# jeremy-collins/sd-video-gen

Measured on AMD Instinct MI355X. Metric: generated frames/sec at 50 DDIM denoise steps, 512x512, higher is better.
Workload: dtype fp16; 1 GPU; configs[2]: 1_16_kitti_L1_64 F=64, 64x64 latents -> 512x512 VAE passes, 50-step DDIM; --denoise --denoise_start_step 0, guidance_scale 0; SD-v1.4 UNet at 64x64 latents, VAE enc/dec at 512x512; clips_per_gpu=56, streams_per_gpu=2, pred_frames=1, global_clips=56, parallelism=clip-sharded dp1, weights=seeded random init (SD v1.4 architecture, 1_16_kitti_L1_64)

## Files before the change

sd-video-gen_amd/csrc/attn.hip:

```cpp
#include "kernels.h"
#include "igemm_epi.h"
#include <cstdlib>

namespace SDNS {

typedef float f32x16 __attribute__((ext_vector_type(16)));

namespace {

constexpr int KVT = 64;
constexpr int VROW = 136;

__device__ __forceinline__ float max3(float a, float b, float c) {
  float r;
  asm("v_max3_f32 %0, %1, %2, %3" : "=v"(r) : "v"(a), "v"(b), "v"(c));
  return r;
}
__device__ __forceinline__ float max_xor32(float v) {
  const auto r = __builtin_amdgcn_permlane32_swap(__float_as_uint(v), __float_as_uint(v), false, false);
  return fmaxf(__uint_as_float(r[0]), __uint_as_float(r[1]));
}

template <int D, int QB, int NSTW, bool BC, bool HV = false>
__global__ void __launch_bounds__(256) attn_kernel(const AttnArgs a) {
// ... 389 lines not shown
      *(uint4*)(sK + tid * KROW + 80) = make_uint4(H16_ONE2, H16_ONE1, 0, 0);
      *(uint4*)(sK + tid * KROW + 96) = make_uint4(0, 0, 0, 0);
    }
    for (int i = tid; i < 24 * 8; i += 256) {
      const int row = 40 + i / 8, pos = i & 7;
      *(uint4*)(sV + row * 128 + pos * 16) = row == 40 ? make_uint4(H16_ONE2, H16_ONE2, H16_ONE2, H16_ONE2) : make_uint4(0, 0, 0, 0);
    }
  }
  __syncthreads();

  f32x16 O[QB][DVT];
  float m_run[QB];
  constexpr float TAU = 6.f;
#pragma unroll
  for (int qb = 0; qb < QB; ++qb) {
#pragma unroll
    for (int i = 0; i < DVT; ++i)
#pragma unroll
      for (int j = 0; j < 16; ++j) O[qb][i][j] = 0.f;
    m_run[qb] = 0.f;
  }

  issue(0);
  if (ntiles > 1) issue(1);
  for (int t = 0; t < ntiles; ++t) {
    if (t + 1 < ntiles) asm volatile("s_waitcnt vmcnt(3)" ::: "memory");
    else asm volatile("s_waitcnt vmcnt(0)" ::: "memory");
    __syncthreads();
    if (t + 2 < ntiles) issue(t + 2);
    const char* const sK = smem + (t % DM_NST) * STAGE;
    const char* const sV = sK + K_BYTES;

    f32x16 S0[QB], S1[QB];
#pragma unroll
    for (int qb = 0; qb < QB; ++qb)
#pragma unroll
      for (int j = 0; j < 16; ++j) { S0[qb][j] = 0.f; S1[qb][j] = 0.f; }
#ifndef ATTN_PRIO
#define ATTN_PRIO 0
#endif
    if (ATTN_PRIO & 1) __builtin_amdgcn_s_setprio(1);
#pragma unroll
    for (int ks = 0; ks < KS; ++ks) {
      const h16x8 a0 = *(const h16x8*)(sK + r * KROW + (ks * 2 + h) * 16);
      const h16x8 a1 = *(const h16x8*)(sK + (32 + r) * KROW + (ks * 2 + h) * 16);
#pragma unroll
      for (int qb = 0; qb < QB; ++qb) {
        S0[qb] = MFMA_32x32x16(a0, qf[qb][ks], S0[qb]);
        S1[qb] = MFMA_32x32x16(a1, qf[qb][ks], S1[qb]);
      }
    }
    if (ATTN_PRIO & 1) __builtin_amdgcn_s_setprio(0);
    uint4 vfr[4 * DVT];
#pragma unroll
    for (int i = 0; i < 4; ++i)
#pragma unroll
      for (int dt = 0; dt < DVT; ++dt) {
        const int row = 32 * dt + r;
        vfr[i * DVT + dt] = *(const uint4*)(sV + row * 128 + (((2 * i + h) ^ ((row >> 1) & 7)) << 4));
      }
    __builtin_amdgcn_sched_barrier(0);
    if (t * KVT + KVT > a.Skv) {
      const int base = t * KVT + 8 * h;
#pragma unroll
      for (int qb = 0; qb < QB; ++qb)
#pragma unroll
        for (int j = 0; j < 16; ++j) {
          const int kv = 16 * (j >> 3) + 4 * ((j >> 2) & 1) + (j & 3);
          if (base + kv >= a.Skv) S0[qb][j] = -INFINITY;
          if (base + 32 + kv >= a.Skv) S1[qb][j] = -INFINITY;
        }
    }
    if (ATTN_PRIO & 4) __builtin_amdgcn_s_setprio(1);
    float mx[QB];
#pragma unroll
    for (int qb = 0; qb < QB; ++qb) {
      float v = fmaxf(S0[qb][0], S1[qb][0]);
#pragma unroll
      for (int j = 1; j < 16; ++j) v = max3(v, S0[qb][j], S1[qb][j]);
      mx[qb] = max_xor32(v);
    }
#pragma unroll
    for (int qb = 0; qb < QB; ++qb) {
      if (t == 0 || __any(mx[qb] > TAU)) {
        const float delta = (t == 0 || mx[qb] > 0.f) ? mx[qb] : 0.f;
        const float alpha = __builtin_amdgcn_exp2f(-delta);
        m_run[qb] += delta;
#pragma unroll
        for (int i = 0; i < DVT; ++i)
#pragma unroll
          for (int j = 0; j < 16; ++j) O[qb][i][j] *= alpha;
#pragma unroll
        for (int j = 0; j < 16; ++j) { S0[qb][j] -= delta; S1[qb][j] -= delta; }
        const float v0 = -m_run[qb];
        const h16 p1 = (h16)v0;
        const float r1 = v0 - (float)p1;
        const h16 p2 = (h16)r1;
        const h16 p3 = (h16)(r1 - (float)p2);
        if (h == 1) { qf[qb][KS - 1][0] = p1; qf[qb][KS - 1][1] = p2; qf[qb][KS - 1][2] = p3; }
      }
#pragma unroll
      for (int j = 0; j < 16; ++j) {
        S0[qb][j] = __builtin_amdgcn_exp2f(S0[qb][j]);
        S1[qb][j] = __builtin_amdgcn_exp2f(S1[qb][j]);
      }
    }
    if (ATTN_PRIO & 4) __builtin_amdgcn_s_setprio(0);
#pragma unroll
    for (int st = 0; st < 2; ++st)
#pragma unroll
      for (int s2 = 0; s2 < 2; ++s2) {
        h16x8 pf[QB];
#pragma unroll
        for (int qb = 0; qb < QB; ++qb)
#pragma unroll
          for (int j = 0; j < 8; ++j) pf[qb][j] = (h16)(st == 0 ? S0[qb][8 * s2 + j] : S1[qb][8 * s2 + j]);
        if (ATTN_PRIO & 2) __builtin_amdgcn_s_setprio(1);
#pragma unroll
        for (int dt = 0; dt < DVT; ++dt) {
          const uint4 v = vfr[(2 * st + s2) * DVT + dt];
#pragma unroll
          for (int qb = 0; qb < QB; ++qb)
            O[qb][dt] = MFMA_32x32x16(*(const h16x8*)&v, pf[qb], O[qb][dt]);
        }
        if (ATTN_PRIO & 2) __builtin_amdgcn_s_setprio(0);
      }
  }

#pragma unroll
  for (int qb = 0; qb < QB; ++qb) {
    const float l_tot = __shfl(O[qb][LT][LR], r + 32 * LH);
    const float inv = 1.f / l_tot;
    const int q = q0 + 32 * qb + r;
    if (q < a.Sq) {
      h16* orow = a.out + (int64_t)b * a.ob + (int64_t)q * a.ldo + head * D;
#pragma unroll
      for (int dt = 0; dt < DVT; ++dt)
#pragma unroll
        for (int g = 0; g < 4; ++g) {
          const int dd = 32 * dt + 8 * g + 4 * h;
          if (dd < D) {
            h16x4 w;
            w[0] = (h16)(O[qb][dt][4 * g + 0] * inv);
            w[1] = (h16)(O[qb][dt][4 * g + 1] * inv);
            w[2] = (h16)(O[qb][dt][4 * g + 2] * inv);
            w[3] = (h16)(O[qb][dt][4 * g + 3] * inv);
            *(h16x4*)(orow + dd) = w;
          }
        }
    }
  }
}

template <int D>
void launch(const AttnPath& p, const AttnArgs& a, hipStream_t s) {
  constexpr bool CAN_BC = (D % 16) == 8;
  if constexpr (D == 40) {
    if (p.kernel == ATTN_DMA40) {
      hipLaunchKernelGGL(attn_dma40_kernel, dim3(cdiv(a.Sq, 256) * a.heads * a.B), dim3(256), 0, s, a);
      return;
    }
  }
  if constexpr (D <= 64) {
    if (p.qb == 2) {
      const dim3 grid(cdiv(a.Sq, 256) * a.heads * a.B);
      if constexpr (CAN_BC) {
        if (p.bc && p.hv) { hipLaunchKernelGGL((attn_kernel<D, 2, 1, true, true>), grid, dim3(256), 0, s, a); return; }
        if (p.bc) { hipLaunchKernelGGL((attn_kernel<D, 2, 1, true>), grid, dim3(256), 0, s, a); return; }
      }
      if (p.nst == 2) hipLaunchKernelGGL((attn_kernel<D, 2, 2, false>), grid, dim3(256), 0, s, a);
      else hipLaunchKernelGGL((attn_kernel<D, 2, 1, false>), grid, dim3(256), 0, s, a);
      return;
    }
  }
  const dim3 grid(cdiv(a.Sq, 128) * a.heads * a.B);
  if constexpr (CAN_BC) {
    if (p.bc) { hipLaunchKernelGGL((attn_kernel<D, 1, 1, true>), grid, dim3(256), 0, s, a); return; }
  }
  if constexpr (D != 160) {
    if (p.nst == 2) { hipLaunchKernelGGL((attn_kernel<D, 1, 2, false>), grid, dim3(256), 0, s, a); return; }
  }
  hipLaunchKernelGGL((attn_kernel<D, 1, 1, false>), grid, dim3(256), 0, s, a);
}

int attn_stages(int d) {
  const int dk = (d + 15) / 16 * 16, dvt = (d + 31) / 32;
  const int stage = KVT * (dk * 2 + 16) + dvt * 32 * VROW;
  return 2 * stage <= 65536 ? 2 : 1;
}

bool attn_d_supported(int d) {
  switch (d) { case 8: case 16: case 32: case 40: case 64: case 80: case 160: return true; default: return false; }
}

bool attn_path_exists(const AttnPath& p) {
  const int d = p.d;
  if (!attn_d_supported(d)) return false;
  if (p.kernel == ATTN_DMA40) return d == 40 && p.qb == 2 && p.nst == 3 && p.bc == 1 && p.hv == 1;
  if (p.kernel != ATTN_REG) return false;
  if (p.qb != 1 && !(p.qb == 2 && d <= 64)) return false;
  if (p.bc) return (d % 16) == 8 && p.bc == 1 && p.nst == 1 && (p.hv == 0 || (p.hv == 1 && p.qb == 2));
  return p.hv == 0 && (p.nst == 1 || (p.nst == 2 && attn_stages(d) == 2));
}

}

AttnPath attention_describe(const AttnArgs& a, const AttnPath* force) {
  SVG_CHECK(attn_d_supported(a.d), "attention: head dim %d unsupported (instantiated: 8, 16, 32, 40, 64, 80, 160)", a.d);
  if (force) {
    SVG_CHECK(force->d == a.d && attn_path_exists(*force), "attention: no instantiation {kernel %d, d %d, QB %d, NST %d, BC %d, HV %d} for d = %d",
              force->kernel, force->d, force->qb, force->nst, force->bc, force->hv, a.d);
    return *force;
  }
  const int nst_env = (int)svg_env_i64("SVG_ATTN_NST", 1);
  const int qb_env = (int)svg_env_i64("SVG_ATTN_QB", 2);
  const int bc_env = (int)svg_env_i64("SVG_ATTN_BC", 1);
  const int hv_env = (int)svg_env_i64("SVG_ATTN_HV", 1);
  const int dma_env = (int)svg_env_i64("SVG_ATTN_DMA", 1);
  const int d = a.d;
  const bool can_bc = (d % 16) == 8;
  AttnPath p;
  p.d = d;
  if (d == 40 && dma_env && qb_env == 2 && bc_env && a.Sq >= 512) {
    p.kernel = ATTN_DMA40; p.qb = 2; p.nst = 3; p.bc = 1; p.hv = 1;
    return p;
  }
  p.qb = (d <= 64 && qb_env == 2 && a.Sq >= 512) ? 2 : 1;
  if (can_bc && bc_env) { p.bc = 1; p.hv = (p.qb == 2 && hv_env) ? 1 : 0; }
  else if (nst_env == 2) p.nst = attn_stages(d);
  return p;
}

void attention(svg_ctx* ctx, const AttnArgs& a, hipStream_t s, const AttnPath* force, AttnPath* ran) {
  SVG_CHECK(a.ldq % 8 == 0 && a.ldk % 8 == 0 && a.ldvt % 8 == 0 && a.ldo % 4 == 0, "attention: strides must be 16-byte aligned");
  SVG_CHECK(a.ldvt >= (a.Skv + 7) / 8 * 8, "attention: V^T rows must be padded to a multiple of 8 keys");
  SVG_CHECK(a.Skv > 0 && a.Sq > 0, "attention: empty");
  const AttnPath p = attention_describe(a, force);
  if (ran) *ran = p;
  if (!SVG_LAUNCHING(ctx)) return;
  char tag[128];
  if (p.kernel == ATTN_DMA40) snprintf(tag, sizeof(tag), "B%d_h%d_Sq%d_Skv%d_d%d_dma40", a.B, a.heads, a.Sq, a.Skv, a.d);
  else snprintf(tag, sizeof(tag), "B%d_h%d_Sq%d_Skv%d_d%d_qb%d_nst%d_bc%d_hv%d", a.B, a.heads, a.Sq, a.Skv, a.d, p.qb, p.nst, p.bc, p.hv);
  ProfScope ps(ctx, PK_ATTN, s, 4.0 * a.B * a.heads * (double)a.Sq * a.Skv * a.d,
               2.0 * a.B * a.heads * ((double)a.Sq * a.d * 2 + (double)a.Skv * a.d * 2), tag);
  switch (a.d) {
    case 8: launch<8>(p, a, s); break;
    case 16: launch<16>(p, a, s); break;
    case 32: launch<32>(p, a, s); break;
    case 40: launch<40>(p, a, s); break;
    case 64: launch<64>(p, a, s); break;
    case 80: launch<80>(p, a, s); break;
    case 160: launch<160>(p, a, s); break;
    default: SVG_CHECK(false, "attention: head dim %d unsupported (instantiated: 8, 16, 32, 40, 64, 80, 160)", a.d);
  }
  check_launch("attention");
}

}
```

sd-video-gen_amd/csrc/kernels.h:

```cpp
#pragma once
#include "common.h"
#include "gemm_tiles.h"

namespace SDNS {

enum AMode { A_DENSE = 0, A_CONV_S1 = 1, A_CONV_S2P1 = 2, A_CONV_S2ASYM = 3, A_CONV_UP2 = 4, A_CONV_SMALLC = 5 };
enum Act { ACT_NONE = 0, ACT_SILU = 1, ACT_GELU = 2, ACT_GEGLU = 3 };

struct GemmArgs {
  const h16* A = nullptr;
  int amode = A_DENSE;
  int lda = 0;
  const h16* A2 = nullptr;
  int lda2 = 0, k_split = 0;
  int H = 0, W = 0, Cin = 0;
  int Ho = 0, Wo = 0;
  const h16* Wt = nullptr;
  int ldb = 0;
  int n_valid = 0;
  void* C = nullptr;
  int ldc = 0;
  int M = 0, N = 0, K = 0;
  int batch = 1;
  int64_t sA = 0, sB = 0, sC = 0;
  float alpha = 1.f;
  const float* bias = nullptr;
  int bias_row = 0;
  const float* bias_bn = nullptr;
  int rows_per_batch = 1;
  int bias_bn_ld = 0;
  const h16* residual = nullptr;
  int ldr = 0;
  int act = ACT_NONE;
  int out_f32 = 0;
  const float* ln_rs = nullptr;
  const float* ln_rm = nullptr;
  const float* ln_s = nullptr;
  int ln_swapped = 0;
  int64_t ln_zstride = 0;
  int splitk = 1;
  float* slabs = nullptr;
  float* gn_part = nullptr;
  float* ln_part = nullptr;
  int ln_tiles = 0;
  int64_t bias_zs = 0;
  h16* vt_out = nullptr;
  int vt_n0 = 0, vt_rows = 0, vt_ld = 0;
  int64_t vt_bs = 0;
  int tn_major = 0;
  int group_m = 0;
  int pp_merge = 0;
  int pp_dma_m = 0;
  int dbg = 0;
  const float* residual_f32 = nullptr;
};

enum GemmFamily { GF_IGEMM = 0, GF_HALO = 1, GF_PP = 2, GF_WS = 3 };
struct GemmPlan {
  int family = GF_IGEMM, bn = 0, splitk = 1;
  int gn_rows = 0;
  int ln_tiles = 0;
  bool operator==(const GemmPlan& o) const { return family == o.family && bn == o.bn && splitk == o.splitk && gn_rows == o.gn_rows && ln_tiles == o.ln_tiles; }
};
GemmPlan gemm_plan(const GemmArgs& g);
void gemm_auto(svg_ctx* ctx, GemmArgs g, const GemmPlan& plan, hipStream_t s, int prof_kind);
void gemm_auto(svg_ctx* ctx, GemmArgs g, hipStream_t s, int prof_kind);
void launch_conv_halo(const GemmArgs& g, int bn, dim3 grid, hipStream_t s);
void launch_gemm_ws(svg_ctx* ctx, const GemmArgs& g, int group_cols, hipStream_t s);
void launch_gemm_pp(const GemmArgs& g, int bn, hipStream_t s);
void gemm_init_device();
void gemm_pp_init_device();
void gemm_ws_init_device();
void conv_halo_init_device();
void ff_fused_init_device();
void xattn_fused_init_device();
void gemm_fp8_init_device();

void quant_mx_h16(svg_ctx* ctx, const h16* x, int ldx, uint8_t* q, uint8_t* sc, int64_t rows, int K, hipStream_t s);
void quant_mx_f32(const float* x, int ldx, uint8_t* q, uint8_t* sc, int64_t rows, int K, hipStream_t s);
bool gemm_fp8_supported(int M, int N, int K);
void gemm_fp8(svg_ctx* ctx, const uint8_t* A, const uint8_t* As, const uint8_t* W, const uint8_t* Ws, const GemmArgs& g, hipStream_t s,
              int* bn_used = nullptr);

bool conv_halo_fp8_supported(int B, int H, int W, int Cin, int N);
void conv_halo_fp8_init_device();
void quant_act_mx(svg_ctx* ctx, const h16* x, int C, uint8_t* q, uint8_t* sc, int64_t P, hipStream_t s);
void pack_conv3x3_mx(const float* w_oihw, uint8_t* q, uint8_t* sc, int O, int I, int Npad, int Cp, hipStream_t s);
struct Fp8ConvPath { int bn = 0, tn_major = 0, workgroups = 0; };
void conv_halo_fp8(svg_ctx* ctx, const uint8_t* A8, const uint8_t* As, const uint8_t* W8, const uint8_t* Ws, int Npad, const GemmArgs& g, hipStream_t s,
                   Fp8ConvPath* path = nullptr);

bool ff_fused_supported(int C, int M);
bool xattn_fused_supported(int C, int heads, int M, int rows_per_sample, int L);
int64_t xattn_kv_pack_elems(int N);
void xattn_pack_q(const float* w, const float* gamma, const float* beta, h16* Wq, float* sq, float* bq, int perm, hipStream_t s);
bool xattn_chain_enabled();
void xattn_pack_o(const float* w, h16* Wo, hipStream_t s);
void xattn_pack_kv(const h16* K, int ldk, int64_t k_bs, const h16* Vt, int ldv, int64_t v_bs, h16* Kp, h16* Vp, int N, int L, hipStream_t s);
void xattn_fused(svg_ctx* ctx, const h16* X, int ldx, const h16* R, int ldr, const h16* Wp, const float* bp, const float* rs, const float* rm,
                 const h16* Wq, const float* sq, const float* bq, const h16* Kp, const h16* Vp, const h16* Wo, const float* bo, h16* out, int ldo,
                 int M, int rows_per_sample, int L, hipStream_t s);
void pack_ff2_perm(const float* w, h16* out, int N, int K, hipStream_t s);
void ff_fused(svg_ctx* ctx, const h16* X, int ldx, const h16* W1, const float* b1, const float* s1,
              const h16* W2p, const float* b2, const h16* residual, int ldr, h16* out, int ldo, int M, hipStream_t s);
void pack_conv3x3(const float* w_oihw, h16* out, int O, int I, int Opad, int Ipad, hipStream_t s);
void pack_linear(const float* w, h16* out, int N, int K, int Npad, hipStream_t s);
void fold_ln_weights(float* w, const float* bias_in, const float* gamma, const float* beta, float* bias_out, int N, int K, hipStream_t s);
void rowsum_h16(const h16* w, float* out, int N, int K, hipStream_t s);
void ln_stats(svg_ctx* ctx, const h16* x, float* rs, float* rm, int M, int C, float eps, hipStream_t s);
void pack_geglu(const float* w, const float* b, h16* wout, float* bout, int F, int K, hipStream_t s);

void ln_finish(svg_ctx* ctx, const float* part, int tiles, float* rs, float* rm, int M, int C, float eps, hipStream_t s);
struct GnStats {
  const float* part = nullptr;
  int tiles_per_sample = 0;
  bool valid() const { return part != nullptr && tiles_per_sample > 0; }
};
void groupnorm(svg_ctx* ctx, const h16* x, int C1, const h16* x2, int C2, const float* gamma,
               const float* beta, h16* out, int B, int HW, int groups, float eps, int silu,
               hipStream_t s, const GnStats* st1 = nullptr, const GnStats* st2 = nullptr);
void groupnorm_f32(svg_ctx* ctx, const float* x, int C, const float* gamma, const float* beta, h16* out, int B, int HW, int groups, float eps,
                   int silu, hipStream_t s, const GnStats* st = nullptr);
enum GnKind { GN_NONE = -1, GN_SMALL = 0, GN_STATS_APPLY = 1, GN_FINISH_APPLY = 2, GN_FINISH_APPLY_MX = 3 };
struct GnPath {
  int kind = GN_NONE, maxch = 0, vw = 0;
  int CV = 0, PL = 0, nchunk = 0, nblk = 0, threads = 0;
};
struct GnShape {
  int C1 = 0, C2 = 0, B = 0, HW = 0, groups = 0;
  bool f32_in = false;
  bool have_stats = false;
  bool mx_out = false;
};
bool groupnorm_mx(svg_ctx* ctx, const h16* x, int C1, const h16* x2, int C2, const float* gamma, const float* beta, uint8_t* q, uint8_t* sc,
                  int B, int HW, int groups, float eps, int silu, hipStream_t s, const GnStats* st1, const GnStats* st2,
                  float* stats_out = nullptr, GnPath* ran = nullptr);
GnPath groupnorm_describe(const GnShape& a, const GnPath* force = nullptr);
void groupnorm_ex(svg_ctx* ctx, const void* x, int C1, const void* x2, int C2, bool f32_in, const float* gamma, const float* beta, h16* out,
                  int B, int HW, int groups, float eps, int silu, hipStream_t s, const GnStats* st1, const GnStats* st2, const GnPath* force,
                  GnPath* ran);
void gn_finish(svg_ctx* ctx, const GnStats& st1, int C1, const GnStats* st2, int C2, float* stats, int B, int HW, int groups, float eps,
               hipStream_t s);
void gn_fold_weights(const float* W, const float* bias, const float* gamma, const float* beta, const float* stats, h16* Wb,
                     float* bb, int B, int N, int C, int groups, hipStream_t s);
void layernorm(svg_ctx* ctx, const h16* x, const float* gamma, const float* beta, h16* out, int M,
               int C, float eps, hipStream_t s);
void softmax_rows(svg_ctx* ctx, const float* s_in, h16* p_out, int64_t rows, int cols, int ld_in,
                  int ld_out, float scale, hipStream_t s);

struct AttnArgs {
  const h16 *q, *k, *vt;
  h16* out;
  int B, heads, Sq, Skv, d;
  int ldq, ldk, ldvt, ldo;
  int64_t qb, kb, vtb, ob;
  float scale;
};
enum AttnKernel { ATTN_REG = 0, ATTN_DMA40 = 1 };
struct AttnPath {
  int kernel = ATTN_REG, d = 0, qb = 1, nst = 1, bc = 0, hv = 0;
};
AttnPath attention_describe(const AttnArgs& a, const AttnPath* force = nullptr);
void attention(svg_ctx* ctx, const AttnArgs& a, hipStream_t s, const AttnPath* force = nullptr, AttnPath* ran = nullptr);
bool vae_attention_supported(int S, int C, int ldqk, int ldvt, int ldo);
bool vae_attention_shape_ok(int S, int C, int ldqk, int ldvt, int ldo);
void vae_attention(svg_ctx* ctx, const h16* q, const h16* k, int ldqk, int64_t qkb, const h16* vt, int ldvt, int64_t vtb, h16* out, int ldo,
                   int64_t ob, int B, int S, int C, hipStream_t s);
void vae_attn_init_device();

void img_to_act(const uint8_t* img, h16* out, int N, int sh, int sw, int H, int W, hipStream_t s);
void act_to_img(const float* x, int ldc, uint8_t* img, float* fout, int N, int h, int w, int oh, int ow,
                hipStream_t s);
void nchw_to_act(const float* x, h16* out, int N, int C, int h, int w, int Cpad, float scale, hipStream_t s);
void nchw_to_actf32(const float* x, float* out, int N, int C, int h, int w, float scale, hipStream_t s);
void actf32_pad_h16(const float* x, int C, h16* out, int Cpad, int64_t P, hipStream_t s);
void actf32_to_nchw(const float* x, int ld, float* out, int N, int C, int h, int w, hipStream_t s);
void pixel_linear_f32(const float* x, int ldx, const float* w, const float* b, float* y, int ldy,
                      int64_t P, int Cin, int Cout, hipStream_t s);
void vae_sample(const float* mom, int ldm, const float* eps_nchw, float* z_nchw, float* mom_nchw, int N,
                int h, int w, hipStream_t s);
void concat_channels(const h16* a, int Ca, const h16* b, int Cb, h16* out, int64_t P, hipStream_t s);
void resize_bilinear_f32(const float* src, float* dst, int P, int h, int w, int oh, int ow, hipStream_t s);
void resize_nearest_u8(const uint8_t* src, uint8_t* dst, int N, int sh, int sw, int C, int dh, int dw,
                       hipStream_t s);
void f32_to_h16(const float* x, h16* y, int64_t n, hipStream_t s);
void h16_to_f32(const h16* x, float* y, int64_t n, hipStream_t s);
void f32_to_h16_x8(const float* x, h16* y, int64_t n, hipStream_t s);
void timestep_embed(const float* t, h16* out, int N, int dim, hipStream_t s);
void fill_f32(float* p, int64_t n, float v, hipStream_t s);

}

void xf_train_init_device();
void xformer_init_device();

struct XfGemmPath { int form, mt, ksplit; };
XfGemmPath xf_gemm_describe(int M, int N, int K);
void xf_gemm(svg_ctx* ctx, const float* X, const float* W, const float* bias, float* Y, int M, int N,
             int K, int act_in, hipStream_t s, const float* residual = nullptr, XfGemmPath* ran = nullptr);
void xf_embed_tokens(const int32_t* ids, const float* tok, const float* pos, float* y, int rows, int T, int d, int vocab, hipStream_t s);
void xf_attention_causal(const float* qkv, float* o, int B, int T, int heads, int hd, hipStream_t s);
void xf_attention_padded(const float* qkv, const int32_t* lens, float* o, int B, int T, int heads, int hd, hipStream_t s);
void xf_embed_bert(const int32_t* ids, const float* word, const float* pos, const float* type0, float* y, int rows, int T, int d, int vocab,
                   hipStream_t s);
void xf_mean_pool_norm(const float* x, const int32_t* lens, float* out, int B, int T, int d, hipStream_t s);
void xf_add_ln(const float* x, const float* r, const float* g, const float* b, float* y, int M, int d,
               float eps, hipStream_t s);
void xf_embed_post(const float* emb, const float* pe, const int32_t* pe_row, const float* text, int d_txt, float* y, int B, int T,
                   int d, float scale, hipStream_t s);
struct XfDrop { const uint64_t* seed; uint32_t site; float p; };
struct XfAdamTensor { float* p; const float* g; float* m; float* v; };
struct XfAdamChunk { int32_t ten; int32_t n; int64_t off; };
void xf_drop_mask(const XfDrop d, float* out, int64_t n, hipStream_t s);
void xf_gemm_tn(const float* dY, int ldy, const float* X, int ldx, float* dW, float* db, int M, int N, int K, int accumulate, hipStream_t s);
int64_t xf_gemm_nn_slab_floats(int M, int N, int K);
int xf_gemm_nn_splits(int N, int K);
void xf_gemm_nn(const float* dY, int ldy, const float* W, float* slabs, float* out, int M, int N, int K, const float* gate, float gate_scale,
                const float* add, hipStream_t s);
void xf_relu_drop(const float* h, float* r, int64_t n, const XfDrop d, hipStream_t s);
void xf_add_ln_train(const float* x, const float* r, const XfDrop dr, const float* g, const float* b, float* y, float* xhat, float* rstd, int M,
                     int d, float eps, hipStream_t s);
void xf_ln_bwd(const float* dy, const float* xhat, const float* rstd, const float* g, float* dz, float* dz_drop, const XfDrop dr, float* dgamma,
               float* dbeta, int M, int d, int accumulate, hipStream_t s);
void xf_embed_post_train(const float* emb, const float* pe, const int32_t* pe_row, const float* text, int d_txt, float* y, int B, int T, int d,
                         float scale, const XfDrop dr, hipStream_t s);
void xf_embed_post_bwd(const float* dy, float* de, int B, int T, int d, int d_img, float scale, const XfDrop dr, hipStream_t s);
void xf_attention_train(const float* q, int ldq, const float* k, const float* v, int ldk, const float* mask, float* o, float* P, int Tq, int Tk,
                        int B, int heads, int hd, const XfDrop dr, hipStream_t s);
void xf_attention_bwd(const float* dout, const float* q, int ldq, const float* k, const float* v, int ldk, const float* P, float* dq, int lddq,
                      float* dk, float* dv, int lddk, int Tq, int Tk, int B, int heads, int hd, const XfDrop dr, hipStream_t s);
void xf_criterion(const float* pred, const float* expected, float* dpred, float* part, float* part2, float* losses, int Tt, int B, int D, int t0,
                  int fh, int fw, float w_mse, float w_l1, float w_gdl, float alpha, float w_nce, float temperature, hipStream_t s);
void xf_adam(const XfAdamTensor* tens, const XfAdamChunk* chunks, int n_chunks, float lr, float beta1, float beta2, float eps, int step,
             float* const* ema, float ema_decay, hipStream_t s);
void xf_grad_norm(const XfAdamTensor* tens, const XfAdamChunk* chunks, int n_chunks, double* part, double* norm, hipStream_t s);
void xf_adamw(const XfAdamTensor* tens, const XfAdamChunk* chunks, int n_chunks, float lr, float beta1, float beta2, float eps, int step,
              float weight_decay, int decoupled, float grad_scale, float max_norm, const double* norm, float* const* ema, float ema_decay,
              hipStream_t s);
void xf_attention(const float* q, int ldq, const float* k, const float* v, int ldk, const float* mask,
                  float* o, int Tq, int Tk, int B, int heads, int hd, hipStream_t s, const float* kpad = nullptr);

int64_t frame_metrics_tiles(int H, int W);
void frame_metrics(const uint8_t* a, const uint8_t* b, int N, int H, int W, double* part_ssim, uint32_t* part_sse, int64_t* sse, double* ssim,
                   float* ssim_map, hipStream_t s);

struct Conv3dArgs {
  const float* x; int B, T, H, W, Cin;
  const float* w;
  const float* bias;
  float* y; int To, Ho, Wo, Cout, ldc, coff;
  int kt, kh, kw, st, sh, sw, pt, ph, pw;
  int relu;
};
void conv3d_launch(const Conv3dArgs& a, hipStream_t s);
void pack_conv3d(const float* w, const float* gamma, const float* beta, const float* mean, const float* var, const float* cbias, float* wout,
                 float* bout, int Cout, int Cin, int Cin_pad, int taps, float eps, hipStream_t s);
void maxpool3d_same(const float* x, float* y, int B, int T, int H, int W, int C, int To, int Ho, int Wo, const int k[3], const int st[3],
                    const int pf[3], hipStream_t s);
void avgpool_thw(const float* x, float* y, int B, int T, int HW, int C, int kt, hipStream_t s);
void time_mean(const float* x, float* y, int B, int To, int C, hipStream_t s);
void ncthw_to_nthwc(const float* x, float* y, int B, int C, int T, int H, int W, int Cp, hipStream_t s);
void fvd_preprocess(const uint8_t* v, float* out, int B, int T, int H, int W, int res, hipStream_t s);
void fd_moments(const float* x, int n, int d, double* mean, double* cov, hipStream_t s);
void sym_eig(double* A, double* V, int d, double* cs, hipStream_t s);
void frechet_distance(const float* x1, int n1, const float* x2, int n2, int d, double* ws, double* out, hipStream_t s);
```

sd-video-gen_amd/csrc/sdnet.cpp:

```cpp
#include "models.h"
#include <algorithm>
#include <cstdlib>

namespace SDNS {

static int64_t chunk_limit() {
  const int64_t full = (1LL << 31) - 1;
  const int64_t v = svg_env_i64("SVG_CHUNK_LIMIT", full);
  return v > 0 && v < full ? v : full;
}

float* keep_f32(svg_ctx* ctx, WeightStore& ws, const std::string& name, int64_t numel) {
  const Weight& w = ws.get(name);
  SVG_CHECK(w.numel == numel, "weight %s has %lld elements, expected %lld", name.c_str(), (long long)w.numel, (long long)numel);
  return w.f32;
}

ConvW load_conv3x3(svg_ctx* ctx, WeightStore& ws, const std::string& prefix, int Cin, int Cout, hipStream_t s, bool fp8) {
  const Weight& w = ws.get(prefix + ".weight", {Cout, Cin, 3, 3});
  ConvW cw;
  cw.Cout = Cout;
  cw.Opad = (int)align_up(Cout, 4);
  cw.Cin = (Cin < 64) ? 8 : Cin;
  SVG_CHECK(Cin <= 8 || Cin % 64 == 0, "conv %s: Cin=%d must be <= 8 or a multiple of 64", prefix.c_str(), Cin);
// ... 78 lines not shown

ConvDims conv_out_dims(int amode, int H, int W) {
  switch (amode) {
    case A_CONV_S1: return {H, W};
    case A_CONV_S2P1: case A_CONV_S2ASYM: return {H / 2, W / 2};
    case A_CONV_UP2: return {2 * H, 2 * W};
    default: throw SvgError("conv3x3: bad mode");
  }
}

bool conv3x3_fp8_ok(const ConvW& cw, int B, int H, int W, bool up2) {
  return cw.w8 != nullptr && conv_halo_fp8_supported(B, up2 ? 2 * H : H, up2 ? 2 * W : W, cw.Cin, cw.Opad);
}

GemmArgs conv3x3_fp8_args(const ConvW& cw, h16* out, int B, int H, int W, int amode, const ConvOpts& o) {
  SVG_CHECK((amode == A_CONV_S1 || amode == A_CONV_UP2) && !o.out_f32 && !o.residual_f32, "conv3x3_fp8: stride 1 (mode %d), 16-bit output and residual only", amode);
  SVG_CHECK(conv3x3_fp8_ok(cw, B, H, W, amode == A_CONV_UP2), "conv3x3_fp8: %d x %dx%d x %d -> %d does not qualify", B, H, W, cw.Cin, cw.Opad);
  const ConvDims d = conv_out_dims(amode, H, W);
  GemmArgs g;
  g.H = H; g.W = W; g.Cin = cw.Cin; g.amode = amode; g.Ho = d.Ho; g.Wo = d.Wo;
  g.K = 9 * cw.Cin; g.M = B * d.Ho * d.Wo; g.N = cw.Opad; g.n_valid = cw.Opad;
  g.bias = cw.b;
  g.bias_bn = o.bias_bn; g.bias_bn_ld = o.bias_bn_ld; g.rows_per_batch = d.Ho * d.Wo;
  g.residual = o.residual; g.ldr = cw.Opad;
  g.C = out; g.ldc = cw.Opad;
  return g;
}

void conv3x3_fp8(svg_ctx* ctx, const uint8_t* x8, const uint8_t* xs, const ConvW& cw, h16* out, int B, int H, int W, int amode, hipStream_t s,
                 const ConvOpts& o) {
  GemmArgs g = conv3x3_fp8_args(cw, out, B, H, W, amode, o);
  attach_gn_emit(g, o.emit, g.Ho * g.Wo, 256);
  conv_halo_fp8(ctx, x8, xs, cw.w8, cw.w8s, cw.Opad, g, s);
}

GemmArgs conv3x3_args(const h16* x, const ConvW& cw, int B, int H, int W, int amode, int out_f32) {
  GemmArgs g;
  g.A = x; g.H = H; g.W = W; g.Cin = cw.Cin;
  g.amode = (cw.Cin == 8) ? A_CONV_SMALLC : amode;
  SVG_CHECK(cw.Cin != 8 || amode == A_CONV_S1, "small-Cin conv supports stride 1 only");
  const ConvDims d = conv_out_dims(amode, H, W);
  g.Ho = d.Ho; g.Wo = d.Wo;
  g.Wt = cw.w; g.ldb = 9 * cw.Cin; g.K = 9 * cw.Cin;
  g.M = B * g.Ho * g.Wo; g.N = cw.Opad; g.n_valid = cw.Opad;
  g.bias = cw.b;
  g.out_f32 = out_f32;
  return g;
}

void conv3x3(svg_ctx* ctx, const h16* x, const ConvW& cw, void* out, int B, int H, int W, int amode, hipStream_t s, const ConvOpts& o) {
  SVG_CHECK(!o.residual_f32 || (o.out_f32 == 2 && !o.residual), "conv3x3: an f32 residual needs the f32-stream output and no 16-bit residual");
  {
    const int up = amode == A_CONV_UP2 ? 4 : 1;
    const int64_t per_img = std::max<int64_t>((int64_t)H * W * std::max(cw.Cin, 8), (int64_t)H * W * up * cw.Opad);
    const int64_t lim = chunk_limit();
    if ((int64_t)B * per_img > lim && B > 1) {
      const int chunk = (int)std::max<int64_t>(1, lim / per_img);
      const ConvDims d = conv_out_dims(amode, H, W);
      ConvOpts c = o;
      c.emit = nullptr;
      for (int b0 = 0; b0 < B; b0 += chunk) {
        const int64_t off = (int64_t)b0 * d.Ho * d.Wo * cw.Opad;
        if (o.bias_bn) c.bias_bn = o.bias_bn + (int64_t)b0 * (o.bias_bn_ld ? o.bias_bn_ld : cw.Opad);
        if (o.residual) c.residual = o.residual + off;
        if (o.residual_f32) c.residual_f32 = o.residual_f32 + off;
        conv3x3(ctx, x + (int64_t)b0 * H * W * cw.Cin, cw, o.out_f32 ? (void*)((float*)out + off) : (void*)((h16*)out + off), std::min(chunk, B - b0),
                H, W, amode, s, c);
      }
      return;
    }
  }
  GemmArgs g = conv3x3_args(x, cw, B, H, W, amode, o.out_f32);
  g.bias_bn = o.bias_bn; g.bias_bn_ld = o.bias_bn_ld; g.rows_per_batch = g.Ho * g.Wo;
  g.residual = o.residual; g.ldr = cw.Opad;
  g.C = out; g.ldc = cw.Opad;
  g.residual_f32 = o.residual_f32;
  const GemmPlan plan = gemm_plan(g);
  attach_gn_emit(g, o.emit, g.Ho * g.Wo, plan.gn_rows);
  gemm_auto(ctx, g, plan, s, PK_CONV3);
}

int conv3x3_halo_width(const ConvW& cw, int B, int H, int W, int amode, int out_f32) {
  const GemmPlan plan = gemm_plan(conv3x3_args(nullptr, cw, B, H, W, amode, out_f32));
  return plan.family == GF_HALO ? plan.bn : 0;
}

void linear(svg_ctx* ctx, const h16* A, int lda, const PackedLinear& pl, void* C, int ldc, int M, hipStream_t s, const LinearOpts& o) {
  if (o.ln) o.ln->tiles = 0;
  SVG_CHECK(!o.residual_f32 || (o.out_f32 == 2 && !o.residual), "linear: an f32 residual needs the f32-stream output and no 16-bit residual");
  SVG_CHECK((pl.ln_s != nullptr) == (o.ln_rs != nullptr), "linear: LayerNorm-folded weights need the row statistics (and only they)");
  {
    const int64_t lim = chunk_limit();
    const int64_t per_row = std::max<int64_t>(lda, std::max(ldc, o.ldr));
    if ((int64_t)M * per_row > lim && M > 1) {
      SVG_CHECK(!o.A2, "linear: a two-source A operand is not split by rows");
      const int chunk = (int)(lim / per_row) & ~255;
      SVG_CHECK(chunk >= 256, "linear: a %lld-element operand limit is below one 256-row slab of %lld-wide rows", (long long)lim, (long long)per_row);
      const int csz = o.out_f32 ? 4 : 2;
      LinearOpts c = o;
      c.emit = nullptr; c.rows_per_sample = 0; c.ln = nullptr;
      for (int m0 = 0; m0 < M; m0 += chunk) {
        if (o.residual) c.residual = o.residual + (int64_t)m0 * o.ldr;
        if (o.residual_f32) c.residual_f32 = o.residual_f32 + (int64_t)m0 * o.ldr;
        if (o.ln_rs) c.ln_rs = o.ln_rs + m0;
        if (o.ln_rm) c.ln_rm = o.ln_rm + m0;
        linear(ctx, A + (int64_t)m0 * lda, lda, pl, (char*)C + (int64_t)m0 * ldc * csz, ldc, std::min(chunk, M - m0), s, c);
      }
      return;
    }
  }
  if (pl.w8 && !o.A2 && !o.ln_rs && o.act != ACT_GEGLU && o.out_f32 != 2 && M >= 1024 && lda == pl.K && gemm_fp8_supported(M, pl.N, pl.K)) {
    ctx->arena.push();
    uint8_t* aq = ctx->arena.get<uint8_t>((int64_t)M * pl.K);
    uint8_t* as = ctx->arena.get<uint8_t>((int64_t)M * (pl.K / 32));
    quant_mx_h16(ctx, A, lda, aq, as, M, pl.K, s);
    GemmArgs g8;
    g8.M = M; g8.N = pl.N; g8.K = pl.K; g8.bias = pl.b; g8.act = o.act; g8.residual = o.residual; g8.ldr = o.ldr; g8.C = C; g8.ldc = ldc; g8.out_f32 = o.out_f32;
    gemm_fp8(ctx, aq, as, pl.w8, pl.w8s, g8, s);
    ctx->arena.pop();
    return;
  }
  GemmArgs g;
  g.ln_rs = o.ln_rs; g.ln_rm = o.ln_rm; g.ln_s = pl.ln_s;
  g.A = A; g.lda = lda; g.Wt = pl.w; g.ldb = pl.K; g.M = M; g.N = pl.N; g.K = pl.K; g.n_valid = pl.N;
  g.bias = pl.b; g.act = o.act; g.residual = o.residual; g.ldr = o.ldr; g.C = C; g.ldc = ldc; g.out_f32 = o.out_f32;
  g.A2 = o.A2; g.lda2 = o.lda2; g.k_split = o.k_split;
  g.residual_f32 = o.residual_f32;
  const GemmPlan plan = gemm_plan(g);
  attach_gn_emit(g, o.emit, o.rows_per_sample, plan.gn_rows);
  plan_ln_emit(g, plan, o.ln);
  gemm_auto(ctx, g, plan, s, PK_GEMM);
}

void vt_proj_into(svg_ctx* ctx, const PackedLinear& wv, const h16* src, int B, int rows, int rows_pad, int K, h16* vt, hipStream_t s,
                  const float* ln_rs, const float* ln_rm) {
  const int C = wv.N;
  GemmArgs g;
  g.A = wv.w; g.lda = K; g.Wt = src; g.ldb = K; g.M = C; g.N = rows_pad; g.n_valid = rows; g.K = K;
  g.batch = B; g.sA = 0; g.sB = (int64_t)rows * K; g.sC = (int64_t)C * rows_pad;
  g.C = vt; g.ldc = rows_pad;
  SVG_CHECK((wv.ln_s != nullptr) == (ln_rs != nullptr), "vt_proj: LayerNorm-folded weights need the token statistics");
  if (wv.b) { g.bias = wv.b; g.bias_row = 1; }
  if (ln_rs) {
    g.ln_rs = ln_rs; g.ln_rm = ln_rm; g.ln_s = wv.ln_s; g.ln_swapped = 1; g.ln_zstride = rows;
  }
  gemm_auto(ctx, g, s, PK_GEMM);
}

void sd_init_device() {
  gemm_init_device();
  gemm_pp_init_device();
  gemm_ws_init_device();
  vae_attn_init_device();
  conv_halo_init_device();
  ff_fused_init_device();
  xattn_fused_init_device();
  gemm_fp8_init_device();
  conv_halo_fp8_init_device();
}

}
```

Before: 18.65 frames/s.

## Add DMA ring-buffered flash attention kernel for head dims 80 and 160

Adds a new attention kernel for d=80 and d=160 that streams K and V^T tiles into LDS through a multi-stage ring of buffer-load-to-LDS DMA transfers (3 stages for d=80, 2 for d=160), using swizzled layouts and no pad columns. The aim is to overlap global loads with MFMA work in the SD UNet's mid/deep self-attention layers, which previously used the register-path kernel. It becomes the default when Skv>96 and bases are aligned. It uses large dynamic LDS with two blocks per CU, which may limit occupancy.

Result: no change. 18.75 frames/s (median of 6 runs) (+0.5%).

```diff
diff --git a/sd-video-gen_amd/csrc/attn.hip b/sd-video-gen_amd/csrc/attn.hip
--- a/sd-video-gen_amd/csrc/attn.hip
+++ b/sd-video-gen_amd/csrc/attn.hip
@@ -565,6 +565,250 @@
   }
 }
 
+template <int D, int QB, int NST>
+__global__ void __launch_bounds__(256, 2) attn_ring_kernel(const AttnArgs a) {
+  static_assert(D % 16 == 0 && (NST == 2 || NST == 3), "no pad columns: the contraction is exactly D wide");
+  constexpr int KS = D / 16, DVT = (D + 31) / 32;
+  constexpr bool ONES = (D % 32) != 0;
+  constexpr int LT = D / 32, LH = ((D % 32) >> 2) & 1, LR = ((D % 32) & 3) + 4 * ((D % 32) >> 3);
+  constexpr int CPR = D / 8;
+  constexpr bool KPAD = (CPR % 4) != 0;
+  constexpr int KCH = KPAD ? CPR + 1 : CPR;
+  constexpr int KROW = KCH * 16;
+  constexpr int K_BYTES = KVT * KROW;
+  constexpr int V_BYTES = DVT * 32 * 128;
+  constexpr int STAGE = K_BYTES + V_BYTES;
+  constexpr int NI = KCH + CPR;
+  constexpr int NJ = (NI + 3) / 4;
+  extern __shared__ __attribute__((aligned(16))) char smem[];
+
+  const int tid = threadIdx.x, lane = tid & 63, wid = __builtin_amdgcn_readfirstlane(tid >> 6);
+  const int r = lane & 31, h = lane >> 5;
+  int b, head, qt;
+  {
+    const int w = xcd_tile(blockIdx.x, gridDim.x);
+    const int nqt = (a.Sq + 128 * QB - 1) / (128 * QB);
+    qt = w % nqt;
+    const int bh = w / nqt;
+    head = bh % a.heads;
+    b = bh / a.heads;
+  }
+  const int q0 = qt * (128 * QB) + wid * (32 * QB);
+  const h16* __restrict__ Q = a.q + (int64_t)b * a.qb + head * D;
+  const h16* __restrict__ Kp = a.k + (int64_t)b * a.kb + head * D;
+  const h16* __restrict__ Vt = a.vt + (int64_t)b * a.vtb + (int64_t)head * D * a.ldvt;
+  const unsigned k_bytes = (unsigned)(((int64_t)a.Skv - 1) * a.ldk * 2 + D * 2);
+  const unsigned v_bytes = (unsigned)(((int64_t)D - 1) * a.ldvt * 2 + ((a.Skv + 7) / 8 * 8) * 2);
+  const v4i srdK = buf_srd(Kp, k_bytes), srdV = buf_srd(Vt, v_bytes);
+  constexpr unsigned OOB = 0x80000000u;
+
+  auto lane_map = [&](int j, unsigned& off, int& kv) {
+    const int idx = wid + 4 * j;
+    if (idx < KCH) {
+      const int slot = idx * 64 + lane;
+      const int rs = slot / KCH, pos = slot - rs * KCH;
+      const int c = KPAD ? pos : pos ^ ((rs >> 2) & 3);
+      const int rho = rs & 31;
+      kv = (rs & 32) + (rho & 16) + ((rho & 4) << 1) + ((rho & 8) >> 1) + (rho & 3);
+      off = c < CPR ? (unsigned)(kv * a.ldk * 2 + c * 16) : OOB;
+    } else {
+      const int slot = (idx - KCH) * 64 + lane;
+      const int row = slot >> 3, pos = slot & 7;
+      const int c = pos ^ ((row >> 1) & 7);
+      kv = 8 * c;
+      off = (unsigned)(row * a.ldvt * 2 + c * 16);
+    }
+  };
+  unsigned voff[NJ];
+#pragma unroll
+  for (int j = 0; j < NJ; ++j) { int kv; lane_map(j, voff[j], kv); }
+  const int nper = (NI - wid + 3) / 4;
+  const unsigned smem_base = (unsigned)(uintptr_t)smem;
+  const int ntiles = (a.Skv + KVT - 1) / KVT;
+  const bool ragged = (a.Skv % KVT) != 0;
+  auto issue = [&](int t) {
+    const unsigned st = smem_base + (unsigned)((t % NST) * STAGE);
+    const bool last = ragged && t == ntiles - 1;
+#pragma unroll
+    for (int j = 0; j < NJ; ++j) {
+      const int idx = wid + 4 * j;
+      if (idx < NI) {
+        unsigned vo = voff[j];
+        if (last) {
+          unsigned o2; int kv;
+          lane_map(j, o2, kv);
+          if (t * KVT + kv >= a.Skv) vo = OOB;
+        }
+        if (idx < KCH) dma16(srdK, vo, t * KVT * a.ldk * 2, __builtin_amdgcn_readfirstlane(st + idx * 1024));
+        else dma16(srdV, vo, t * KVT * 2, __builtin_amdgcn_readfirstlane(st + K_BYTES + (idx - KCH) * 1024));
+      }
+    }
+  };
+
+  const float c = a.scale * 1.4426950408889634f;
+  h16x8 qf[QB][KS];
+#pragma unroll
+  for (int qb = 0; qb < QB; ++qb) {
+    const int q = q0 + 32 * qb + r;
+#pragma unroll
+    for (int ks = 0; ks < KS; ++ks) {
+      uint4 v = make_uint4(0, 0, 0, 0);
+      if (q < a.Sq) v = *(const uint4*)(Q + (int64_t)q * a.ldq + ks * 16 + h * 8);
+      qf[qb][ks] = *(h16x8*)&v;
+    }
+  }
+  if (ONES) {
+#pragma unroll
+    for (int st = 0; st < NST; ++st) {
+      char* const sV = smem + st * STAGE + K_BYTES;
+      for (int i = tid; i < (DVT * 32 - D) * 8; i += 256) {
+        const int row = D + i / 8, pos = i & 7;
+        *(uint4*)(sV + row * 128 + pos * 16) = row == D ? make_uint4(H16_ONE2, H16_ONE2, H16_ONE2, H16_ONE2) : make_uint4(0, 0, 0, 0);
+      }
+    }
+  }
+  __syncthreads();
+
+  f32x16 O[QB][DVT];
+  float m_run[QB], l_run[QB], mc[QB];
+#pragma unroll
+  for (int qb = 0; qb < QB; ++qb) {
+#pragma unroll
+    for (int i = 0; i < DVT; ++i)
+#pragma unroll
+      for (int j = 0; j < 16; ++j) O[qb][i][j] = 0.f;
+    m_run[qb] = -1e30f; l_run[qb] = 0.f; mc[qb] = m_run[qb] * c;
+  }
+
+  issue(0);
+  if (NST == 3 && ntiles > 1) issue(1);
+  for (int t = 0; t < ntiles; ++t) {
+    if (NST == 3 && t + 1 < ntiles) wait_vm(nper);
+    else asm volatile("s_waitcnt vmcnt(0)" ::: "memory");
+    __syncthreads();
+    if (t + NST - 1 < ntiles) issue(t + NST - 1);
+    const char* const sK = smem + (t % NST) * STAGE;
+    const char* const sV = sK + K_BYTES;
+
+    f32x16 S0[QB], S1[QB];
+#pragma unroll
+    for (int qb = 0; qb < QB; ++qb)
+#pragma unroll
+      for (int j = 0; j < 16; ++j) { S0[qb][j] = 0.f; S1[qb][j] = 0.f; }
+#pragma unroll
+    for (int ks = 0; ks < KS; ++ks) {
+      const int ch = ks * 2 + h;
+      const int p0 = KPAD ? ch : ch ^ ((r >> 2) & 3);
+      const h16x8 a0 = *(const h16x8*)(sK + r * KROW + p0 * 16);
+      const h16x8 a1 = *(const h16x8*)(sK + (32 + r) * KROW + p0 * 16);
+#pragma unroll
+      for (int qb = 0; qb < QB; ++qb) {
+        S0[qb] = MFMA_32x32x16(a0, qf[qb][ks], S0[qb]);
+        S1[qb] = MFMA_32x32x16(a1, qf[qb][ks], S1[qb]);
+      }
+    }
+    if (t * KVT + KVT > a.Skv) {
+      const int base = t * KVT + 8 * h;
+#pragma unroll
+      for (int qb = 0; qb < QB; ++qb)
+#pragma unroll
+        for (int j = 0; j < 16; ++j) {
+          const int kv = 16 * (j >> 3) + 4 * ((j >> 2) & 1) + (j & 3);
+          if (base + kv >= a.Skv) S0[qb][j] = -INFINITY;
+          if (base + 32 + kv >= a.Skv) S1[qb][j] = -INFINITY;
+        }
+    }
+    float mx[QB];
+#pragma unroll
+    for (int qb = 0; qb < QB; ++qb) {
+      float v = fmaxf(S0[qb][0], S1[qb][0]);
+#pragma unroll
+      for (int j = 1; j < 16; ++j) v = max3(v, S0[qb][j], S1[qb][j]);
+      mx[qb] = max_xor32(v);
+    }
+#pragma unroll
+    for (int qb = 0; qb < QB; ++qb) {
+      if (__any(mx[qb] > m_run[qb])) {
+        const float m_new = fmaxf(m_run[qb], mx[qb]);
+        const float alpha = __builtin_amdgcn_exp2f((m_run[qb] - m_new) * c);
+        m_run[qb] = m_new;
+        mc[qb] = m_new * c;
+        if (!ONES) l_run[qb] *= alpha;
+#pragma unroll
+        for (int i = 0; i < DVT; ++i)
+#pragma unroll
+          for (int j = 0; j < 16; ++j) O[qb][i][j] *= alpha;
+      }
+    }
+#pragma unroll
+    for (int qb = 0; qb < QB; ++qb) {
+#pragma unroll
+      for (int j = 0; j < 16; ++j) {
+        S0[qb][j] = __builtin_amdgcn_exp2f(fmaf(S0[qb][j], c, -mc[qb]));
+        S1[qb][j] = __builtin_amdgcn_exp2f(fmaf(S1[qb][j], c, -mc[qb]));
+      }
+      if (!ONES) {
+        float psum = 0.f;
+#pragma unroll
+        for (int j = 0; j < 16; ++j) psum += S0[qb][j] + S1[qb][j];
+        l_run[qb] += psum;
+      }
+    }
+#pragma unroll
+    for (int st = 0; st < 2; ++st)
+#pragma unroll
+      for (int s2 = 0; s2 < 2; ++s2) {
+        h16x8 pf[QB];
+#pragma unroll
+        for (int qb = 0; qb < QB; ++qb)
+#pragma unroll
+          for (int j = 0; j < 8; ++j) pf[qb][j] = (h16)(st == 0 ? S0[qb][8 * s2 + j] : S1[qb][8 * s2 + j]);
+        const int i = 2 * st + s2;
+#pragma unroll
+        for (int dt = 0; dt < DVT; ++dt) {
+          const int row = 32 * dt + r;
+          const uint4 v = *(const uint4*)(sV + row * 128 + (((2 * i + h) ^ ((row >> 1) & 7)) << 4));
+#pragma unroll
+          for (int qb = 0; qb < QB; ++qb)
+            O[qb][dt] = MFMA_32x32x16(*(const h16x8*)&v, pf[qb], O[qb][dt]);
+        }
+      }
+  }
+
+#pragma unroll
+  for (int qb = 0; qb < QB; ++qb) {
+    float l_tot;
+    if (ONES) l_tot = __shfl(O[qb][LT][LR], r + 32 * LH);
+    else l_tot = l_run[qb] + __shfl_xor(l_run[qb], 32);
+    const float inv = 1.f / l_tot;
+    const int q = q0 + 32 * qb + r;
+    if (q < a.Sq) {
+      h16* orow = a.out + (int64_t)b * a.ob + (int64_t)q * a.ldo + head * D;
+#pragma unroll
+      for (int dt = 0; dt < DVT; ++dt)
+#pragma unroll
+        for (int g = 0; g < 4; ++g) {
+          const int dd = 32 * dt + 8 * g + 4 * h;
+          if (dd < D) {
+            h16x4 w;
+            w[0] = (h16)(O[qb][dt][4 * g + 0] * inv);
+            w[1] = (h16)(O[qb][dt][4 * g + 1] * inv);
+            w[2] = (h16)(O[qb][dt][4 * g + 2] * inv);
+            w[3] = (h16)(O[qb][dt][4 * g + 3] * inv);
+            *(h16x4*)(orow + dd) = w;
+          }
+        }
+    }
+  }
+}
+
+template <int D, int NST>
+constexpr int ring_lds() {
+  constexpr int cpr = D / 8, kch = (cpr % 4) != 0 ? cpr + 1 : cpr;
+  return NST * (KVT * kch * 16 + (D + 31) / 32 * 32 * 128);
+}
+constexpr int ring_nst(int d) { return d == 80 ? 3 : 2; }
+
 template <int D>
 void launch(const AttnPath& p, const AttnArgs& a, hipStream_t s) {
   constexpr bool CAN_BC = (D % 16) == 8;
@@ -574,6 +818,19 @@
       return;
     }
   }
+  if constexpr (D == 80 || D == 160) {
+    if (p.kernel == ATTN_RING) {
+      constexpr int NST = ring_nst(D), LDS = ring_lds<D, NST>();
+      if constexpr (D == 80) {
+        if (p.qb == 2) {
+          hipLaunchKernelGGL((attn_ring_kernel<D, 2, NST>), dim3(cdiv(a.Sq, 256) * a.heads * a.B), dim3(256), LDS, s, a);
+          return;
+        }
+      }
+      hipLaunchKernelGGL((attn_ring_kernel<D, 1, NST>), dim3(cdiv(a.Sq, 128) * a.heads * a.B), dim3(256), LDS, s, a);
+      return;
+    }
+  }
   if constexpr (D <= 64) {
     if (p.qb == 2) {
       const dim3 grid(cdiv(a.Sq, 256) * a.heads * a.B);
@@ -610,12 +867,24 @@
   const int d = p.d;
   if (!attn_d_supported(d)) return false;
   if (p.kernel == ATTN_DMA40) return d == 40 && p.qb == 2 && p.nst == 3 && p.bc == 1 && p.hv == 1;
+  if (p.kernel == ATTN_RING)
+    return (d == 80 || d == 160) && (p.qb == 1 || (p.qb == 2 && d == 80)) && p.nst == ring_nst(d) && p.bc == 0 && p.hv == 0;
   if (p.kernel != ATTN_REG) return false;
   if (p.qb != 1 && !(p.qb == 2 && d <= 64)) return false;
   if (p.bc) return (d % 16) == 8 && p.bc == 1 && p.nst == 1 && (p.hv == 0 || (p.hv == 1 && p.qb == 2));
   return p.hv == 0 && (p.nst == 1 || (p.nst == 2 && attn_stages(d) == 2));
 }
 
+bool attn_bases_aligned(const AttnArgs& a) {
+  return (((uintptr_t)a.q | (uintptr_t)a.k | (uintptr_t)a.vt) & 15) == 0 && (a.qb % 8) == 0 && (a.kb % 8) == 0 && (a.vtb % 8) == 0;
+}
+
+}
+
+void attn_init_device() {
+  HIP_OK(hipFuncSetAttribute((const void*)attn_ring_kernel<80, 2, 3>, hipFuncAttributeMaxDynamicSharedMemorySize, ring_lds<80, 3>()));
+  HIP_OK(hipFuncSetAttribute((const void*)attn_ring_kernel<80, 1, 3>, hipFuncAttributeMaxDynamicSharedMemorySize, ring_lds<80, 3>()));
+  HIP_OK(hipFuncSetAttribute((const void*)attn_ring_kernel<160, 1, 2>, hipFuncAttributeMaxDynamicSharedMemorySize, ring_lds<160, 2>()));
 }
 
 AttnPath attention_describe(const AttnArgs& a, const AttnPath* force) {
@@ -630,12 +899,17 @@
   const int bc_env = (int)svg_env_i64("SVG_ATTN_BC", 1);
   const int hv_env = (int)svg_env_i64("SVG_ATTN_HV", 1);
   const int dma_env = (int)svg_env_i64("SVG_ATTN_DMA", 1);
+  const int ring_env = (int)svg_env_i64("SVG_ATTN_RING", 1);
   const int d = a.d;
   const bool can_bc = (d % 16) == 8;
   AttnPath p;
   p.d = d;
   if (d == 40 && dma_env && qb_env == 2 && bc_env && a.Sq >= 512) {
     p.kernel = ATTN_DMA40; p.qb = 2; p.nst = 3; p.bc = 1; p.hv = 1;
+    return p;
+  }
+  if ((d == 80 || d == 160) && ring_env && a.Skv > 96 && attn_bases_aligned(a)) {
+    p.kernel = ATTN_RING; p.qb = (d == 80 && a.Sq >= 512) ? 2 : 1; p.nst = ring_nst(d);
     return p;
   }
   p.qb = (d <= 64 && qb_env == 2 && a.Sq >= 512) ? 2 : 1;
@@ -652,7 +926,9 @@
   if (ran) *ran = p;
   if (!SVG_LAUNCHING(ctx)) return;
   char tag[128];
+  SVG_CHECK(p.kernel != ATTN_RING || attn_bases_aligned(a), "attention: the ring kernels need 16-byte aligned q, k, vt and batch strides");
   if (p.kernel == ATTN_DMA40) snprintf(tag, sizeof(tag), "B%d_h%d_Sq%d_Skv%d_d%d_dma40", a.B, a.heads, a.Sq, a.Skv, a.d);
+  else if (p.kernel == ATTN_RING) snprintf(tag, sizeof(tag), "B%d_h%d_Sq%d_Skv%d_d%d_ring_qb%d_nst%d", a.B, a.heads, a.Sq, a.Skv, a.d, p.qb, p.nst);
   else snprintf(tag, sizeof(tag), "B%d_h%d_Sq%d_Skv%d_d%d_qb%d_nst%d_bc%d_hv%d", a.B, a.heads, a.Sq, a.Skv, a.d, p.qb, p.nst, p.bc, p.hv);
   ProfScope ps(ctx, PK_ATTN, s, 4.0 * a.B * a.heads * (double)a.Sq * a.Skv * a.d,
                2.0 * a.B * a.heads * ((double)a.Sq * a.d * 2 + (double)a.Skv * a.d * 2), tag);
diff --git a/sd-video-gen_amd/csrc/kernels.h b/sd-video-gen_amd/csrc/kernels.h
--- a/sd-video-gen_amd/csrc/kernels.h
+++ b/sd-video-gen_amd/csrc/kernels.h
@@ -156,7 +156,7 @@
   int64_t qb, kb, vtb, ob;
   float scale;
 };
-enum AttnKernel { ATTN_REG = 0, ATTN_DMA40 = 1 };
+enum AttnKernel { ATTN_REG = 0, ATTN_DMA40 = 1, ATTN_RING = 2 };
 struct AttnPath {
   int kernel = ATTN_REG, d = 0, qb = 1, nst = 1, bc = 0, hv = 0;
 };
@@ -167,6 +167,7 @@
 void vae_attention(svg_ctx* ctx, const h16* q, const h16* k, int ldqk, int64_t qkb, const h16* vt, int ldvt, int64_t vtb, h16* out, int ldo,
                    int64_t ob, int B, int S, int C, hipStream_t s);
 void vae_attn_init_device();
+void attn_init_device();
 
 void img_to_act(const uint8_t* img, h16* out, int N, int sh, int sw, int H, int W, hipStream_t s);
 void act_to_img(const float* x, int ldc, uint8_t* img, float* fout, int N, int h, int w, int oh, int ow,
diff --git a/sd-video-gen_amd/csrc/sdnet.cpp b/sd-video-gen_amd/csrc/sdnet.cpp
--- a/sd-video-gen_amd/csrc/sdnet.cpp
+++ b/sd-video-gen_amd/csrc/sdnet.cpp
@@ -254,6 +254,7 @@
   gemm_pp_init_device();
   gemm_ws_init_device();
   vae_attn_init_device();
+  attn_init_device();
   conv_halo_init_device();
   ff_fused_init_device();
   xattn_fused_init_device();
```
